# showlab/VideoSwap

Measured on NVIDIA H100. Metric: denoise-steps/sec, 16f 512^2 SD1.5 UNet3D (CFG UNet fwd + CFG combine + DDIM step), higher is better.
Workload: dtype f16

## Files before the change

### videoswap_b200/csrc/common.cuh

```cuda
#pragma once
#include <cuda.h>
#include <cuda_fp16.h>
#include <cuda_runtime.h>
#include <stdint.h>
#include <stdio.h>

namespace vs {

void set_error(const char* fmt, ...);
const char* last_error();

#define VS_CHECK_CUDA(expr)                                                                         \
  do {                                                                                              \
    cudaError_t _e = (expr);                                                                        \
    if (_e != cudaSuccess) {                                                                        \
      vs::set_error("%s:%d CUDA error %s: %s", __FILE__, __LINE__, #expr, cudaGetErrorString(_e)); \
      return 1;                                                                                     \
    }                                                                                               \
  } while (0)

#define VS_REQUIRE(cond, ...)                \
  do {                                       \
    if (!(cond)) {                           \
      vs::set_error(__VA_ARGS__);            \
      return 2;                              \
    }                                        \
  } while (0)

int make_tmap_f16(CUtensorMap* out, const void* base, int rank, const uint64_t* dims, const uint64_t* strides_bytes,
                  const uint32_t* box, int swizzle );

int num_sms();
int get_option(const char* name);

#ifdef __CUDACC__
template <typename... KArgs, typename... Args>
int launch_pdl(void (*kernel)(KArgs...), dim3 grid, dim3 block, size_t smem, cudaStream_t st, int cluster_x, Args&&... args) {
  cudaLaunchConfig_t cfg = {};
  cfg.gridDim = grid;
  cfg.blockDim = block;
  cfg.dynamicSmemBytes = smem;
  cfg.stream = st;
  cudaLaunchAttribute attr[2];
  int n = 0;
  if (get_option("pdl") != 0) {
    attr[n].id = cudaLaunchAttributeProgrammaticStreamSerialization;
    attr[n].val.programmaticStreamSerializationAllowed = 1;
    ++n;
  }
  if (cluster_x > 1) {
    attr[n].id = cudaLaunchAttributeClusterDimension;
    attr[n].val.clusterDim.x = cluster_x;
    attr[n].val.clusterDim.y = 1;
    attr[n].val.clusterDim.z = 1;
    ++n;
  }
  cfg.attrs = attr;
  cfg.numAttrs = n;
  VS_CHECK_CUDA(cudaLaunchKernelEx(&cfg, kernel, static_cast<KArgs>(args)...));
  return 0;
}
#endif

enum ProfCat { PC_GEMM = 0, PC_CONV = 1, PC_ATTN = 2, PC_TATTN = 3, PC_GROUPNORM = 4, PC_LAYERNORM = 5, PC_OTHER = 6, PC_COUNT = 7 };
struct ProfScope {
  ProfScope(cudaStream_t st, int cat, double work, int nlaunch = 1, long long m = 0, int n = 0, int k = 0);
  ~ProfScope();
  cudaStream_t st_; int idx_;
};
void prof_enable(bool on);
void prof_reset();
int prof_collect(int cat, double* ms, double* work, long long* count);
int prof_dump(const char* path);
long long launch_count();
void count_launch(int n);

#ifdef __CUDACC__
__device__ __forceinline__ uint32_t smem_u32(const void* p) { return (uint32_t)__cvta_generic_to_shared(p); }

__device__ __forceinline__ void mbar_init(uint32_t bar, uint32_t count) {
  asm volatile("mbarrier.init.shared::cta.b64 [%0], %1;" ::"r"(bar), "r"(count) : "memory");
}
__device__ __forceinline__ void fence_barrier_init() {
  asm volatile("fence.mbarrier_init.release.cluster;" ::: "memory");
}
__device__ __forceinline__ void fence_proxy_async() { asm volatile("fence.proxy.async.shared::cta;" ::: "memory"); }
__device__ __forceinline__ void mbar_expect_tx(uint32_t bar, uint32_t bytes) {
  asm volatile("mbarrier.arrive.expect_tx.shared::cta.b64 _, [%0], %1;" ::"r"(bar), "r"(bytes) : "memory");
}
__device__ __forceinline__ void mbar_arrive(uint32_t bar) {
  asm volatile("mbarrier.arrive.shared::cta.b64 _, [%0];" ::"r"(bar) : "memory");
}
__device__ __forceinline__ bool mbar_try_wait(uint32_t bar, uint32_t parity) {
  uint32_t ok;
  asm volatile(
      "{\n\t.reg .pred p;\n\t"
      "mbarrier.try_wait.parity.shared::cta.b64 p, [%1], %2;\n\t"
      "selp.u32 %0, 1, 0, p;\n\t}"
      : "=r"(ok)
      : "r"(bar), "r"(parity)
      : "memory");
  return ok != 0;
}
__device__ __forceinline__ void mbar_wait(uint32_t bar, uint32_t parity) {
  if (mbar_try_wait(bar, parity)) return;
  uint32_t spins = 0;
  while (!mbar_try_wait(bar, parity)) {
    if (++spins > (1u << 25)) __trap();
  }
}

__device__ __forceinline__ void prefetch_tmap(const CUtensorMap* m) {
  asm volatile("prefetch.tensormap [%0];" ::"l"(reinterpret_cast<uint64_t>(m)) : "memory");
}
__device__ __forceinline__ void tma_load_2d(uint32_t dst, const CUtensorMap* m, uint32_t bar, int c0, int c1) {
  asm volatile(
      "cp.async.bulk.tensor.2d.shared::cluster.global.mbarrier::complete_tx::bytes [%0], [%1, {%3, %4}], [%2];"
      ::"r"(dst), "l"(reinterpret_cast<uint64_t>(m)), "r"(bar), "r"(c0), "r"(c1)
      : "memory");
}
__device__ __forceinline__ void tma_load_4d(uint32_t dst, const CUtensorMap* m, uint32_t bar, int c0, int c1, int c2,
                                            int c3) {
  asm volatile(
      "cp.async.bulk.tensor.4d.shared::cluster.global.mbarrier::complete_tx::bytes [%0], [%1, {%3, %4, %5, %6}], [%2];"
      ::"r"(dst), "l"(reinterpret_cast<uint64_t>(m)), "r"(bar), "r"(c0), "r"(c1), "r"(c2), "r"(c3)
      : "memory");
}

__device__ __forceinline__ bool elect_one() {
  uint32_t pred;
  asm volatile(
      "{\n\t.reg .pred P;\n\t"
      "elect.sync _|P, 0xffffffff;\n\t"
      "selp.u32 %0, 1, 0, P;\n\t}"
      : "=r"(pred));
  return pred != 0;
}

__device__ __forceinline__ uint32_t cluster_ctarank() {
  uint32_t r;
  asm volatile("mov.u32 %0, %%cluster_ctarank;" : "=r"(r));
  return r;
}
__device__ __forceinline__ void cluster_sync_all() {
  asm volatile("barrier.cluster.arrive.release.aligned;" ::: "memory");
  asm volatile("barrier.cluster.wait.acquire.aligned;" ::: "memory");
}
__device__ __forceinline__ uint32_t mapa_shared(uint32_t addr, uint32_t rank) {
  uint32_t r;
  asm volatile("mapa.shared::cluster.u32 %0, %1, %2;" : "=r"(r) : "r"(addr), "r"(rank));
  return r;
}
__device__ __forceinline__ void named_bar_sync(int id, int nthreads) {
  asm volatile("bar.sync %0, %1;" ::"r"(id), "r"(nthreads) : "memory");
}
__device__ __forceinline__ void named_bar_arrive(int id, int nthreads) {
  asm volatile("bar.arrive %0, %1;" ::"r"(id), "r"(nthreads) : "memory");
}

__device__ __forceinline__ void pdl_trigger() { asm volatile("griddepcontrol.launch_dependents;" ::: "memory"); }
__device__ __forceinline__ void pdl_wait() { asm volatile("griddepcontrol.wait;" ::: "memory"); }

template <int N>
__device__ __forceinline__ void setmaxnreg_dec() { asm volatile("setmaxnreg.dec.sync.aligned.u32 %0;" ::"n"(N)); }
template <int N>
__device__ __forceinline__ void setmaxnreg_inc() { asm volatile("setmaxnreg.inc.sync.aligned.u32 %0;" ::"n"(N)); }

__device__ __forceinline__ void wgmma_fence() { asm volatile("wgmma.fence.sync.aligned;" ::: "memory"); }
__device__ __forceinline__ void wgmma_commit() { asm volatile("wgmma.commit_group.sync.aligned;" ::: "memory"); }
template <int N>
__device__ __forceinline__ void wgmma_wait() { asm volatile("wgmma.wait_group.sync.aligned %0;" ::"n"(N) : "memory"); }

__device__ __forceinline__ uint64_t gmma_desc_sw128(uint32_t smem_addr) {
  uint64_t d = 0;
  d |= (uint64_t)((smem_addr & 0x3FFFF) >> 4);
  d |= (uint64_t)1 << 16;
  d |= (uint64_t)(1024 >> 4) << 32;
  d |= (uint64_t)1 << 62;
  return d;
}
__device__ __forceinline__ uint64_t gmma_desc_sw128_mn(uint32_t smem_addr, uint32_t lbo_bytes) {
  uint64_t d = 0;
  d |= (uint64_t)((smem_addr & 0x3FFFF) >> 4);
  d |= (uint64_t)((lbo_bytes >> 4) & 0x3FFF) << 16;
  d |= (uint64_t)(1024 >> 4) << 32;
  d |= (uint64_t)1 << 62;
  return d;
}

#define VS_R8(i) "+f"(d[i]), "+f"(d[i + 1]), "+f"(d[i + 2]), "+f"(d[i + 3]), "+f"(d[i + 4]), "+f"(d[i + 5]), "+f"(d[i + 6]), "+f"(d[i + 7])
template <int N>
__device__ __forceinline__ void wgmma_ss(float* d, uint64_t da, uint64_t db, uint32_t scale_d);
#define VS_REGS_0_31 "%0,%1,%2,%3,%4,%5,%6,%7,%8,%9,%10,%11,%12,%13,%14,%15,%16,%17,%18,%19,%20,%21,%22,%23,%24,%25,%26,%27,%28,%29,%30,%31"
#define VS_REGS_32_63 "%32,%33,%34,%35,%36,%37,%38,%39,%40,%41,%42,%43,%44,%45,%46,%47,%48,%49,%50,%51,%52,%53,%54,%55,%56,%57,%58,%59,%60,%61,%62,%63"
#define VS_REGS_64_79 "%64,%65,%66,%67,%68,%69,%70,%71,%72,%73,%74,%75,%76,%77,%78,%79"
#define VS_REGS_80_127 "%80,%81,%82,%83,%84,%85,%86,%87,%88,%89,%90,%91,%92,%93,%94,%95,%96,%97,%98,%99,%100,%101,%102,%103,%104,%105,%106,%107,%108,%109,%110,%111,%112,%113,%114,%115,%116,%117,%118,%119,%120,%121,%122,%123,%124,%125,%126,%127"
#define VS_WGMMA_SS(N, REGS, IA, IB, IS, ...)                                                                     \
  template <>                                                                                                     \
  __device__ __forceinline__ void wgmma_ss<N>(float* d, uint64_t da, uint64_t db, uint32_t scale_d) {           \
    asm volatile("{\n\t.reg .pred p;\n\tsetp.ne.b32 p, %" #IS ", 0;\n\t"                                         \
                 "wgmma.mma_async.sync.aligned.m64n" #N "k16.f32.f16.f16 {" REGS "}, %" #IA ", %" #IB ", p, 1, 1, 0, 0;\n\t}" \
                 : __VA_ARGS__                                                                                    \
                 : "l"(da), "l"(db), "r"(scale_d));                                                               \
  }
VS_WGMMA_SS(64, VS_REGS_0_31, 32, 33, 34, VS_R8(0), VS_R8(8), VS_R8(16), VS_R8(24))
VS_WGMMA_SS(128, VS_REGS_0_31 "," VS_REGS_32_63, 64, 65, 66, VS_R8(0), VS_R8(8), VS_R8(16), VS_R8(24), VS_R8(32), VS_R8(40),
            VS_R8(48), VS_R8(56))
VS_WGMMA_SS(160, VS_REGS_0_31 "," VS_REGS_32_63 "," VS_REGS_64_79, 80, 81, 82, VS_R8(0), VS_R8(8), VS_R8(16), VS_R8(24),
            VS_R8(32), VS_R8(40), VS_R8(48), VS_R8(56), VS_R8(64), VS_R8(72))
VS_WGMMA_SS(256, VS_REGS_0_31 "," VS_REGS_32_63 "," VS_REGS_64_79 "," VS_REGS_80_127, 128, 129, 130, VS_R8(0), VS_R8(8),
            VS_R8(16), VS_R8(24), VS_R8(32), VS_R8(40), VS_R8(48), VS_R8(56), VS_R8(64), VS_R8(72), VS_R8(80), VS_R8(88),
            VS_R8(96), VS_R8(104), VS_R8(112), VS_R8(120))
#undef VS_WGMMA_SS
#undef VS_REGS_0_31
#undef VS_REGS_32_63
#undef VS_REGS_64_79
#undef VS_REGS_80_127
template <int TB = 0>
__device__ __forceinline__ void wgmma_m64n16(float* d, uint64_t da, uint64_t db, uint32_t scale_d) {
  asm volatile(
      "{\n\t.reg .pred p;\n\tsetp.ne.b32 p, %10, 0;\n\t"
      "wgmma.mma_async.sync.aligned.m64n16k16.f32.f16.f16 {%0,%1,%2,%3,%4,%5,%6,%7}, %8, %9, p, 1, 1, 0, %11;\n\t}"
      : VS_R8(0)
      : "l"(da), "l"(db), "r"(scale_d), "n"(TB));
}
template <int TB = 0>
__device__ __forceinline__ void wgmma_m64n64_rs(float* d, const uint32_t* a, uint64_t db, uint32_t scale_d) {
  asm volatile(
      "{\n\t.reg .pred p;\n\tsetp.ne.b32 p, %37, 0;\n\t"
      "wgmma.mma_async.sync.aligned.m64n64k16.f32.f16.f16 "
      "{%0,%1,%2,%3,%4,%5,%6,%7,%8,%9,%10,%11,%12,%13,%14,%15,%16,%17,%18,%19,%20,%21,%22,%23,%24,%25,%26,%27,%28,%29,%30,%31}, "
      "{%32,%33,%34,%35}, %36, p, 1, 1, %38;\n\t}"
      : VS_R8(0), VS_R8(8), VS_R8(16), VS_R8(24)
      : "r"(a[0]), "r"(a[1]), "r"(a[2]), "r"(a[3]), "l"(db), "r"(scale_d), "n"(TB));
}
template <int TB = 0>
__device__ __forceinline__ void wgmma_m64n16_rs(float* d, const uint32_t* a, uint64_t db, uint32_t scale_d) {
  asm volatile(
      "{\n\t.reg .pred p;\n\tsetp.ne.b32 p, %13, 0;\n\t"
      "wgmma.mma_async.sync.aligned.m64n16k16.f32.f16.f16 {%0,%1,%2,%3,%4,%5,%6,%7}, {%8,%9,%10,%11}, %12, p, 1, 1, %14;\n\t}"
      : VS_R8(0)
      : "r"(a[0]), "r"(a[1]), "r"(a[2]), "r"(a[3]), "l"(db), "r"(scale_d), "n"(TB));
}
#undef VS_R8

__device__ __forceinline__ float silu_f(float x) { return __fdividef(x, 1.f + __expf(-x)); }
__device__ __forceinline__ float gelu_erf_f(float x) { return 0.5f * x * (1.f + erff(x * 0.70710678118654752f)); }
__device__ __forceinline__ float gelu_erf_fast(float x) {
  const float z = fabsf(x) * 0.70710678118654752f;
  float t;
  asm("rcp.approx.ftz.f32 %0, %1;" : "=f"(t) : "f"(fmaf(0.3275911f, z, 1.f)));
  float poly = fmaf(1.061405429f, t, -1.453152027f);
  poly = fmaf(poly, t, 1.421413741f);
  poly = fmaf(poly, t, -0.284496736f);
  poly = fmaf(poly, t, 0.254829592f);
  poly *= t;
  float e;
  asm("ex2.approx.ftz.f32 %0, %1;" : "=f"(e) : "f"(-1.4426950408889634f * z * z));
  const float erf_abs = fmaf(-poly, e, 1.f);
  const float erf_s = copysignf(erf_abs, x);
  return 0.5f * x * (1.f + erf_s);
}
__device__ __forceinline__ float gelu_sig(float x) {
  const float xc = fminf(fmaxf(x, -5.f), 5.f);
  const float u = xc * xc;
  float q = fmaf(u, 2.47135360e-05f, 7.37690930e-04f);
  q = fmaf(q, u, -1.05988323e-01f);
  q = fmaf(q, u, -2.30164247e+00f);
  float e;
  asm("ex2.approx.ftz.f32 %0, %1;" : "=f"(e) : "f"(xc * q));
  return __fdividef(x, 1.f + e);
}
#endif

}
```

### videoswap_b200/csrc/gemm.cu

```cuda
#include "common.cuh"
#include "kernels.h"

namespace vs {

namespace {

constexpr int BM = 128;
constexpr int WG_M = 64;
constexpr int BK = 64;
constexpr int A_STAGE_BYTES = BM * BK * 2;
constexpr uint64_t A_HALF_DESC = (WG_M * BK * 2) >> 4;
constexpr int GEMM_THREADS = 384;
constexpr int SMEM_LIMIT = 227 * 1024;
constexpr int EPI_COLS = 32;
constexpr int EPI_WARP_BYTES = 16 * 64;
constexpr int EPI_BYTES = 8 * EPI_WARP_BYTES;
constexpr int PRODUCER_REGS = 40, CONSUMER_REGS = 232;
enum { EPI_F_GEGLU = 1, EPI_F_RES = 2, EPI_F_RV = 4, EPI_F_LN = 8, EPI_F_LNOUT = 16 };

struct GemmParams {
  CUtensorMap tmA, tmA2, tmB;
  int M, N;
  int num_kb;
  int kb_per_tap;
  int kb_src1;
  int taps;
  int a_rank;
  int nimg, H, W, TH, TW, TN, tiles_x, tiles_y;
  int tap_x0, tap_y0, tap_w;
  int osy, osx, ooy, oox, OH, OW;
  int tw_log, thw_log;
  int m_tiles, n_tiles;
  const float* bias;
  const float* rowvec;
  int ldrv;
  int pix_per_batch;
  int rv_mod;
  const float2* ln_stats;
  const float* ln_u;
  const float2* ln_parts;
  int ln_nparts;
  float ln_inv_c;
  float2* ln_sums_out;
  const __half* residual;
  int ldr;
  __half* out;
  int ldc;
  int staged;
  int stages;
};

template <int BN>
struct Cfg {
  static constexpr bool COOP = BN > 160;
  static constexpr int HALVES = COOP ? 1 : 2;
  static constexpr int B_STAGE_BYTES = BN * BK * 2;
  static constexpr int STAGE_BYTES = A_STAGE_BYTES + B_STAGE_BYTES;
  static constexpr int STAGES_RAW = (SMEM_LIMIT - 2048 - EPI_BYTES) / STAGE_BYTES;
  static constexpr int STAGES = STAGES_RAW > 12 ? 12 : STAGES_RAW;
  static constexpr int SMEM_BYTES = STAGES * STAGE_BYTES + EPI_BYTES + 1024  + 256 ;
  static_assert(B_STAGE_BYTES % 1024 == 0, "B stage must keep 1024-byte alignment for SWIZZLE_128B");
  static_assert(STAGES >= 3, "pipeline too shallow");
  static_assert(BN % 32 == 0 && BN <= 256, "wgmma N");
};

__device__ __forceinline__ uint32_t sw64_off(int row, int chunk) {
  return (uint32_t)(row * 64 + ((chunk ^ ((row >> 1) & 3)) << 4));
}

template <int BN, int EPI>
__global__ void __launch_bounds__(GEMM_THREADS, 1) gemm_tc_kernel(const __grid_constant__ GemmParams p) {
  using C = Cfg<BN>;
  constexpr bool GEGLU = (EPI & EPI_F_GEGLU) != 0, HAS_RES = (EPI & EPI_F_RES) != 0, HAS_RV = (EPI & EPI_F_RV) != 0;
  constexpr bool LN = (EPI & EPI_F_LN) != 0;
  constexpr bool LNOUT = (EPI & EPI_F_LNOUT) != 0;
  extern __shared__ uint8_t smem_raw[];
  const uint32_t smem_base = (smem_u32(smem_raw) + 1023u) & ~1023u;
  const uint32_t epi_base = smem_base + C::STAGES * C::STAGE_BYTES;
  const uint32_t bar_base = epi_base + EPI_BYTES;
  auto full_bar = [&](int s) { return bar_base + 8u * s; };
  auto empty_bar = [&](int s) { return bar_base + 8u * (C::STAGES + s); };

  const int warp = threadIdx.x >> 5;
  const int lane = threadIdx.x & 31;
  const int wg = threadIdx.x >> 7;
  const int nst = (p.stages > 0 && p.stages < C::STAGES) ? p.stages : C::STAGES;
  const int total_tiles = p.m_tiles * p.n_tiles;

  if (threadIdx.x == 0) {
    prefetch_tmap(&p.tmA);
    prefetch_tmap(&p.tmB);
    if (p.kb_src1 < p.kb_per_tap) prefetch_tmap(&p.tmA2);
    for (int s = 0; s < C::STAGES; ++s) {
      mbar_init(full_bar(s), 1);
      mbar_init(empty_bar(s), C::COOP ? 8 : 4);
    }
    fence_barrier_init();
  }
  __syncthreads();
  pdl_trigger();
  pdl_wait();

  if (wg == 0) {
    setmaxnreg_dec<PRODUCER_REGS>();
    if (warp != 0) return;
    const int num_kb = p.num_kb, kb_per_tap = p.kb_per_tap, kb_src1 = p.kb_src1;
    const bool conv = p.a_rank == 4;
    const int tap_x0 = p.tap_x0, tap_x1 = p.tap_x0 + p.tap_w;
    uint32_t pr_s = 0, pr_ph = 0;
    for (int t = blockIdx.x; t < total_tiles; t += gridDim.x) {
      const int m_tile = t / p.n_tiles, n_tile = t % p.n_tiles;
      int x0 = 0, y0 = 0, i0 = 0;
      if (conv) {
        x0 = (m_tile % p.tiles_x) * p.TW;
        y0 = ((m_tile / p.tiles_x) % p.tiles_y) * p.TH;
        i0 = (m_tile / (p.tiles_x * p.tiles_y)) * p.TN;
      }
      const int n0 = n_tile * BN;
      const int m0 = m_tile * BM;
      int kcoord = 0;
      int dy = p.tap_y0, dx = tap_x0;
      int r = 0;
      for (int kb = 0; kb < num_kb; ++kb) {
        mbar_wait(empty_bar(pr_s), pr_ph ^ 1);
        if (elect_one()) {
          const uint32_t fb = full_bar(pr_s);
          const uint32_t a_dst = smem_base + pr_s * C::STAGE_BYTES;
          const bool first = r < kb_src1;
          const CUtensorMap* tm = first ? &p.tmA : &p.tmA2;
          const int c = (first ? r : r - kb_src1) * BK;
          mbar_expect_tx(fb, C::STAGE_BYTES);
          if (conv) tma_load_4d(a_dst, tm, fb, c, x0 + dx, y0 + dy, i0);
          else tma_load_2d(a_dst, tm, fb, c, m0);
          tma_load_2d(a_dst + A_STAGE_BYTES, &p.tmB, fb, kcoord, n0);
        }
        __syncwarp();
        kcoord += BK;
        if (++r == kb_per_tap) {
          r = 0;
          if (++dx == tap_x1) { dx = tap_x0; ++dy; }
        }
        if (++pr_s == (uint32_t)nst) { pr_s = 0; pr_ph ^= 1; }
      }
    }
    return;
  }

  setmaxnreg_inc<CONSUMER_REGS>();
  const int g = wg - 1;
  const int wq = warp & 3;
  const int q = lane & 3;
  const int rbase = 16 * wq + (lane >> 2);
  const uint32_t stage_buf = epi_base + (uint32_t)(warp - 4) * EPI_WARP_BYTES;
  const bool has_bias = p.bias != nullptr;
  const bool staged = p.staged != 0;
  const int num_kb = p.num_kb;
  auto tile_pixel = [&](int m_tile, int row) -> int {
    if (p.a_rank == 4) {
      const int x0 = (m_tile % p.tiles_x) * p.TW;
      const int y0 = ((m_tile / p.tiles_x) % p.tiles_y) * p.TH;
      const int i0 = (m_tile / (p.tiles_x * p.tiles_y)) * p.TN;
      const int ti = row >> p.thw_log, rem = row & ((1 << p.thw_log) - 1);
      const int y = y0 + (rem >> p.tw_log), x = x0 + (rem & (p.TW - 1)), img = i0 + ti;
      return ((img < p.nimg) && (y < p.H) && (x < p.W)) ? (img * p.OH + y * p.osy + p.ooy) * p.OW + x * p.osx + p.oox : -1;
    }
    const int px = m_tile * BM + row;
    return px < p.M ? px : -1;
  };

  const int bar_mine = 1 + g, bar_other = 2 - g;
  float acc[C::HALVES][BN / 2];
  uint32_t s = 0, ph = 0;
  for (int t = blockIdx.x, j = 0; t < total_tiles; t += gridDim.x, ++j) {
    const int m_tile = t / p.n_tiles, n_tile = t % p.n_tiles;
    if (!C::COOP && (j & 1) != g) {
      const uint32_t sn = s + (uint32_t)num_kb;
      ph ^= (sn / (uint32_t)nst) & 1u;
      s = sn % (uint32_t)nst;
      continue;
    }
    if (!C::COOP && j > 0) named_bar_sync(bar_mine, 256);
    uint32_t prev = 0;
    for (int kb = 0; kb < num_kb; ++kb) {
      mbar_wait(full_bar(s), ph);
      wgmma_fence();
      const uint32_t a_addr = smem_base + s * C::STAGE_BYTES;
      const uint64_t da = gmma_desc_sw128(a_addr) + (C::COOP ? (uint64_t)g * A_HALF_DESC : 0);
      const uint64_t db = gmma_desc_sw128(a_addr + A_STAGE_BYTES);
#pragma unroll
      for (int k = 0; k < BK / 16; ++k) {
#pragma unroll
        for (int hh = 0; hh < C::HALVES; ++hh)
          wgmma_ss<BN>(acc[hh], da + hh * A_HALF_DESC + 2 * k, db + 2 * k, (kb | k) != 0 ? 1u : 0u);
      }
      wgmma_commit();
      if (kb > 0) {
        wgmma_wait<1>();
        if (lane == 0) mbar_arrive(empty_bar(prev));
      }
      prev = s;
      if (++s == (uint32_t)nst) { s = 0; ph ^= 1; }
    }
    if (!C::COOP && t + (int)gridDim.x < total_tiles) named_bar_arrive(bar_other, 256);
    wgmma_wait<0>();
    if (lane == 0) mbar_arrive(empty_bar(prev));

    const int n0 = n_tile * BN;
#pragma unroll
    for (int hh = 0; hh < C::HALVES; ++hh) {
      const int r0 = WG_M * (C::COOP ? g : hh) + rbase;
      int pix[2];
      pix[0] = tile_pixel(m_tile, r0);
      pix[1] = tile_pixel(m_tile, r0 + 8);
      const float* rv[2] = {nullptr, nullptr};
      if (HAS_RV || !staged) {
#pragma unroll
        for (int h = 0; h < 2; ++h) {
          if (p.rowvec != nullptr && pix[h] >= 0) {
            int ri = pix[h] / p.pix_per_batch;
            if (p.rv_mod > 0) ri %= p.rv_mod;
            rv[h] = p.rowvec + (long long)ri * p.ldrv + n0;
          }
        }
      }
      if (staged) {
        constexpr int OC = GEGLU ? BN / 2 : BN;
        const int oc0 = n_tile * OC;
        const int nsub = (p.N - n0 < BN ? (GEGLU ? (p.N - n0) / 2 : p.N - n0) : OC) / EPI_COLS;
        float la[2] = {1.f, 1.f}, lb[2] = {0.f, 0.f};
        if (LN) {
#pragma unroll
          for (int h = 0; h < 2; ++h) {
            if (pix[h] < 0) continue;
            if (p.ln_nparts > 0) {
              float S = 0.f, Q = 0.f;
              for (int k = 0; k < p.ln_nparts; ++k) {
                const float2 v = __ldg(p.ln_parts + (long long)k * p.M + pix[h]);
                S += v.x; Q += v.y;
              }
              const float mean = S * p.ln_inv_c;
              la[h] = rsqrtf(fmaxf(fmaf(-mean, mean, Q * p.ln_inv_c), 0.f) + 1e-5f);
              lb[h] = -mean * la[h];
            } else {
              const float2 st2 = __ldg(p.ln_stats + pix[h]);
              la[h] = st2.x; lb[h] = st2.y;
            }
          }
        }
        float rs[2] = {0.f, 0.f}, rq[2] = {0.f, 0.f};
        __half* orow[2];
        const __half* rrow[2];
#pragma unroll
        for (int h = 0; h < 2; ++h) {
          const long long px = pix[h] >= 0 ? pix[h] : 0;
          orow[h] = p.out + px * p.ldc + oc0 + q * 8;
          rrow[h] = HAS_RES ? p.residual + px * p.ldr + oc0 + q * 8 : nullptr;
        }
#pragma unroll
        for (int sb = 0; sb < OC / EPI_COLS; ++sb) {
          if (sb >= nsub) break;
          uint4 rr[2];
          if (HAS_RES) {
#pragma unroll
            for (int h = 0; h < 2; ++h) rr[h] = __ldg(reinterpret_cast<const uint4*>(rrow[h] + sb * EPI_COLS));
          }
#pragma unroll
          for (int jj = 0; jj < 4; ++jj) {
            const int j = 4 * sb + jj;
            const int c = 8 * j + 2 * q;
            float2 b = has_bias ? __ldg(reinterpret_cast<const float2*>(p.bias + n0 + c)) : make_float2(0.f, 0.f);
            float2 u = LN ? __ldg(reinterpret_cast<const float2*>(p.ln_u + n0 + c)) : make_float2(0.f, 0.f);
            float2 bg = make_float2(0.f, 0.f), ug = make_float2(0.f, 0.f);
            if (GEGLU) {
              bg = __ldg(reinterpret_cast<const float2*>(p.bias + n0 + BN / 2 + c));
              if (LN) ug = __ldg(reinterpret_cast<const float2*>(p.ln_u + n0 + BN / 2 + c));
            }
#pragma unroll
            for (int h = 0; h < 2; ++h) {
              float f0 = acc[hh][4 * j + 2 * h], f1 = acc[hh][4 * j + 2 * h + 1];
              if (GEGLU) {
                float g0 = acc[hh][4 * (j + BN / 16) + 2 * h], g1 = acc[hh][4 * (j + BN / 16) + 2 * h + 1];
                float bv0 = b.x, bv1 = b.y, bg0 = bg.x, bg1 = bg.y;
                if (LN) {
                  bv0 = fmaf(lb[h], u.x, bv0); bv1 = fmaf(lb[h], u.y, bv1);
                  bg0 = fmaf(lb[h], ug.x, bg0); bg1 = fmaf(lb[h], ug.y, bg1);
                  f0 *= la[h]; f1 *= la[h]; g0 *= la[h]; g1 *= la[h];
                }
                f0 = (f0 + bv0) * gelu_sig(g0 + bg0);
                f1 = (f1 + bv1) * gelu_sig(g1 + bg1);
              } else {
                if (LN) {
                  f0 = fmaf(la[h], f0, fmaf(lb[h], u.x, b.x));
                  f1 = fmaf(la[h], f1, fmaf(lb[h], u.y, b.y));
                } else if (has_bias) {
                  f0 += b.x; f1 += b.y;
                }
                if (HAS_RV && rv[h] != nullptr) {
                  const float2 r2 = __ldg(reinterpret_cast<const float2*>(rv[h] + c));
                  f0 += r2.x; f1 += r2.y;
                }
              }
              const __half2 hv = __floats2half2_rn(f0, f1);
              asm volatile("st.shared.b32 [%0], %1;" ::"r"(stage_buf + sw64_off((lane >> 2) + 8 * h, jj) + 4 * q),
                           "r"(*reinterpret_cast<const uint32_t*>(&hv)) : "memory");
            }
          }
          __syncwarp();
#pragma unroll
          for (int h = 0; h < 2; ++h) {
            uint4 o;
            asm volatile("ld.shared.v4.b32 {%0,%1,%2,%3}, [%4];" : "=r"(o.x), "=r"(o.y), "=r"(o.z), "=r"(o.w)
                         : "r"(stage_buf + sw64_off((lane >> 2) + 8 * h, q)));
            if (HAS_RES) {
              __half2* oh = reinterpret_cast<__half2*>(&o);
              const __half2* rh = reinterpret_cast<const __half2*>(&rr[h]);
#pragma unroll
              for (int t = 0; t < 4; ++t) oh[t] = __hadd2(oh[t], rh[t]);
            }
            if (pix[h] >= 0) *reinterpret_cast<uint4*>(orow[h] + sb * EPI_COLS) = o;
            if (LNOUT) {
              const __half2* oh = reinterpret_cast<const __half2*>(&o);
              const float2 a = __half22float2(oh[0]), b2 = __half22float2(oh[1]), c2 = __half22float2(oh[2]), d2 = __half22float2(oh[3]);
              rs[h] += ((a.x + a.y) + (b2.x + b2.y)) + ((c2.x + c2.y) + (d2.x + d2.y));
              float q0 = fmaf(a.x, a.x, a.y * a.y), q1 = fmaf(b2.x, b2.x, b2.y * b2.y);
              float q2 = fmaf(c2.x, c2.x, c2.y * c2.y), q3 = fmaf(d2.x, d2.x, d2.y * d2.y);
              rq[h] += (q0 + q1) + (q2 + q3);
            }
          }
          __syncwarp();
        }
        if (LNOUT) {
#pragma unroll
          for (int h = 0; h < 2; ++h) {
            rs[h] += __shfl_xor_sync(0xffffffffu, rs[h], 1); rq[h] += __shfl_xor_sync(0xffffffffu, rq[h], 1);
            rs[h] += __shfl_xor_sync(0xffffffffu, rs[h], 2); rq[h] += __shfl_xor_sync(0xffffffffu, rq[h], 2);
            if (q == 0 && pix[h] >= 0) p.ln_sums_out[(long long)n_tile * p.M + pix[h]] = make_float2(rs[h], rq[h]);
          }
        }
      } else {
#pragma unroll
        for (int j = 0; j < BN / 8; ++j) {
#pragma unroll
          for (int e = 0; e < 4; ++e) {
            const int h = e >> 1, c = 8 * j + 2 * q + (e & 1), n = n0 + c;
            if (n < p.N && pix[h] >= 0) {
              float f = acc[hh][4 * j + e];
              if (has_bias) f += p.bias[n];
              if (rv[h]) f += rv[h][c];
              if (p.residual) f += __half2float(p.residual[(long long)pix[h] * p.ldr + n]);
              p.out[(long long)pix[h] * p.ldc + n] = __float2half_rn(f);
            }
          }
        }
      }
    }
  }
}

struct ConvTile { int tw, th, tn; };

ConvTile pick_conv_tile(int nimg, int H, int W) {
  ConvTile best{1, 1, BM};
  long long best_cost = -1;
  for (int tw = 1; tw <= BM; tw *= 2) {
    for (int th = 1; tw * th <= BM; th *= 2) {
      const int tn = BM / (tw * th);
      if (tw > 256 || th > 256 || tn > 256) continue;
      const long long cost = (long long)((W + tw - 1) / tw) * tw * ((H + th - 1) / th) * th * ((nimg + tn - 1) / tn) * tn;
      if (best_cost < 0 || cost < best_cost || (cost == best_cost && tw > best.tw)) {
        best_cost = cost;
        best = ConvTile{tw, th, tn};
      }
    }
  }
  return best;
}

template <int BN, int EPI>
int launch(cudaStream_t st, const GemmParams& p) {
  using C = Cfg<BN>;
  static bool configured = false;
  if (!configured) {
    VS_CHECK_CUDA(cudaFuncSetAttribute(gemm_tc_kernel<BN, EPI>, cudaFuncAttributeMaxDynamicSharedMemorySize, C::SMEM_BYTES));
    configured = true;
  }
  const int total = p.m_tiles * p.n_tiles;
  int ctas = num_sms();
  const int cap = get_option("gemm_ctas");
  if (cap > 0 && cap < ctas) ctas = cap;
  return launch_pdl(gemm_tc_kernel<BN, EPI>, dim3(total < ctas ? total : ctas), dim3(GEMM_THREADS), C::SMEM_BYTES, st, 1, p);
}

template <int BN>
int launch_linear(cudaStream_t st, const GemmParams& p) {
  const int epi = (p.residual ? EPI_F_RES : 0) | (p.rowvec ? EPI_F_RV : 0) | ((p.ln_stats || p.ln_parts) ? EPI_F_LN : 0) |
                  (p.ln_sums_out ? EPI_F_LNOUT : 0);
  switch (epi) {
    case EPI_F_LNOUT: return launch<BN, EPI_F_LNOUT>(st, p);
    case EPI_F_LNOUT | EPI_F_RES: return launch<BN, EPI_F_LNOUT | EPI_F_RES>(st, p);
    case EPI_F_LN: return launch<BN, EPI_F_LN>(st, p);
    case EPI_F_LN | EPI_F_RV: return launch<BN, EPI_F_LN | EPI_F_RV>(st, p);
    case 0: return launch<BN, 0>(st, p);
    case EPI_F_RES: return launch<BN, EPI_F_RES>(st, p);
    case EPI_F_RV: return launch<BN, EPI_F_RV>(st, p);
    case EPI_F_RES | EPI_F_RV: return launch<BN, EPI_F_RES | EPI_F_RV>(st, p);
    default: set_error("gemm_tc: unsupported epilogue combination 0x%x", epi); return 2;
  }
}

int pick_bn(int m_tiles, int N, int num_kb) {
  if (N <= 64) return 64;
  int best = 128;
  long long best_cost = -1;
  const int cand[3] = {128, 160, 256};
  for (int i = 0; i < 3; ++i) {
    const int bn = cand[i];
    if (bn != 128 && N % bn != 0) continue;
    const long long tiles = (long long)m_tiles * ((N + bn - 1) / bn);
    const long long waves = (tiles + num_sms() - 1) / num_sms();
    const long long cost = waves * (16 + bn / 8);
    if (best_cost < 0 || cost < best_cost || (cost == best_cost && num_kb >= 40)) {
      best_cost = cost;
      best = bn;
    }
  }
  return best;
}

int ilog2(int v) { int l = 0; while ((1 << l) < v) ++l; return l; }

}

int gemm_n_tiles(const GemmArgs& a) {
  if (a.taps != 1) return 0;
  int bn = a.force_bn;
  if (a.mode == EPI_GEGLU) bn = 2 * kGegluGranule;
  else if (bn == 0) bn = pick_bn((a.M + BM - 1) / BM, a.N, (a.K1 + BK - 1) / BK + a.K2 / BK);
  return (a.N + bn - 1) / bn;
}

int gemm_tc(cudaStream_t st, const GemmArgs& a) {
  VS_REQUIRE(a.A && a.Bw && a.out, "gemm_tc: null pointer");
  VS_REQUIRE(a.taps == 1 || a.taps == 9 || a.taps == 4, "gemm_tc: taps must be 1, 9 (3x3) or 4 (2x2 sub-pixel)");
  VS_REQUIRE(a.K1 % 8 == 0 && a.K2 % 8 == 0, "gemm_tc: K must be a multiple of 8 (TMA 16-byte strides)");
  VS_REQUIRE((long long)a.M * (a.ldc > a.ldr ? a.ldc : a.ldr) < (1LL << 40) && a.M < (1 << 30), "gemm_tc: M too large");
  const bool two = a.A2 != nullptr && a.K2 > 0;
  if (two || a.taps != 1) VS_REQUIRE(a.K1 % BK == 0 && a.K2 % BK == 0, "gemm_tc: concat/conv sources need C %% 64 == 0 (got %d,%d)", a.K1, a.K2);
  GemmParams p;
  memset(&p, 0, sizeof(p));
  const int Ktap = a.K1 + (two ? a.K2 : 0);
  const int Ktot = Ktap * a.taps;
  p.taps = a.taps;
  p.kb_src1 = (a.K1 + BK - 1) / BK;
  p.kb_per_tap = p.kb_src1 + (two ? a.K2 / BK : 0);
  p.num_kb = p.kb_per_tap * a.taps;
  p.M = a.M;
  p.N = a.N;
  p.bias = a.bias;
  p.rowvec = a.rowvec;
  p.ldrv = a.ldrv > 0 ? a.ldrv : a.N;
  p.pix_per_batch = a.pix_per_batch > 0 ? a.pix_per_batch : 1;
  p.rv_mod = a.rv_mod;
  p.ln_stats = reinterpret_cast<const float2*>(a.ln_stats);
  p.ln_u = a.ln_u;
  p.ln_parts = reinterpret_cast<const float2*>(a.ln_parts);
  p.ln_nparts = a.ln_parts ? a.ln_nparts : 0;
  p.ln_inv_c = 1.f / (float)(a.K1 + a.K2);
  p.ln_sums_out = reinterpret_cast<float2*>(a.ln_sums_out);
  if (a.ln_parts) VS_REQUIRE(a.ln_stats == nullptr && a.ln_nparts >= 1 && a.ln_nparts <= 16 && a.taps == 1, "gemm_tc: bad LayerNorm partial-sum input");
  if (a.ln_stats || a.ln_parts) VS_REQUIRE(a.ln_u != nullptr && a.bias != nullptr && a.residual == nullptr, "gemm_tc: folded LayerNorm needs u and c vectors and no residual");
  if (a.ln_sums_out) VS_REQUIRE(a.taps == 1 && a.mode == EPI_LINEAR && a.rowvec == nullptr && !a.ln_stats && !a.ln_parts,
                                "gemm_tc: row statistics output is implemented for plain linear layers (+ bias / residual)");
  p.residual = a.residual;
  p.ldr = a.ldr;
  p.out = a.out;
  p.ldc = a.ldc;
  p.stages = get_option("gemm_stages");

  if (a.taps != 1) {
    VS_REQUIRE(a.nimg > 0 && a.H > 0 && a.W > 0 && a.M == a.nimg * a.H * a.W, "gemm_tc: bad conv geometry");
    p.a_rank = 4;
    if (a.taps == 9) { p.tap_x0 = p.tap_y0 = -1; p.tap_w = 3; p.osy = p.osx = 1; p.ooy = p.oox = 0; p.OH = a.H; p.OW = a.W; }
    else {
      VS_REQUIRE((a.sub_py | 1) == 1 && (a.sub_px | 1) == 1, "gemm_tc: sub-pixel parity must be 0 or 1");
      p.tap_y0 = a.sub_py - 1; p.tap_x0 = a.sub_px - 1; p.tap_w = 2;
      p.osy = p.osx = 2; p.ooy = a.sub_py; p.oox = a.sub_px; p.OH = 2 * a.H; p.OW = 2 * a.W;
    }
    const ConvTile t = pick_conv_tile(a.nimg, a.H, a.W);
    p.nimg = a.nimg; p.H = a.H; p.W = a.W; p.TW = t.tw; p.TH = t.th; p.TN = t.tn;
    p.tw_log = ilog2(t.tw);
    p.thw_log = ilog2(t.tw * t.th);
    p.tiles_x = (a.W + t.tw - 1) / t.tw;
    p.tiles_y = (a.H + t.th - 1) / t.th;
    p.m_tiles = p.tiles_x * p.tiles_y * ((a.nimg + t.tn - 1) / t.tn);
    const uint32_t box[4] = {BK, (uint32_t)t.tw, (uint32_t)t.th, (uint32_t)t.tn};
    {
      const uint64_t dims[4] = {(uint64_t)a.K1, (uint64_t)a.W, (uint64_t)a.H, (uint64_t)a.nimg};
      const uint64_t str[3] = {(uint64_t)a.lda1 * 2, (uint64_t)a.lda1 * 2 * a.W, (uint64_t)a.lda1 * 2 * a.W * a.H};
      if (make_tmap_f16(&p.tmA, a.A, 4, dims, str, box, 1)) return 3;
    }
    if (two) {
      const uint64_t dims[4] = {(uint64_t)a.K2, (uint64_t)a.W, (uint64_t)a.H, (uint64_t)a.nimg};
      const uint64_t str[3] = {(uint64_t)a.lda2 * 2, (uint64_t)a.lda2 * 2 * a.W, (uint64_t)a.lda2 * 2 * a.W * a.H};
      if (make_tmap_f16(&p.tmA2, a.A2, 4, dims, str, box, 1)) return 3;
    }
  } else {
    p.a_rank = 2;
    p.m_tiles = (a.M + BM - 1) / BM;
    const uint32_t box[2] = {BK, BM};
    {
      const uint64_t dims[2] = {(uint64_t)a.K1, (uint64_t)a.M};
      const uint64_t str[1] = {(uint64_t)a.lda1 * 2};
      if (make_tmap_f16(&p.tmA, a.A, 2, dims, str, box, 1)) return 3;
    }
    if (two) {
      const uint64_t dims[2] = {(uint64_t)a.K2, (uint64_t)a.M};
      const uint64_t str[1] = {(uint64_t)a.lda2 * 2};
      if (make_tmap_f16(&p.tmA2, a.A2, 2, dims, str, box, 1)) return 3;
    }
  }

  int bn = a.force_bn;
  if (a.mode == EPI_GEGLU) {
    bn = 2 * kGegluGranule;
    VS_REQUIRE(a.N % bn == 0, "gemm_tc: GEGLU needs N %% %d == 0 (N=%d)", bn, a.N);
    VS_REQUIRE(a.bias != nullptr && a.residual == nullptr && a.rowvec == nullptr, "gemm_tc: GEGLU takes a bias only");
  } else if (bn == 0) {
    bn = pick_bn(p.m_tiles, a.N, p.num_kb);
  }
  VS_REQUIRE(bn == 64 || bn == 128 || bn == 160 || bn == 256, "gemm_tc: unsupported BLOCK_N %d", bn);
  p.n_tiles = (a.N + bn - 1) / bn;
  {
    const uint64_t dims[2] = {(uint64_t)Ktot, (uint64_t)a.N};
    const uint64_t str[1] = {(uint64_t)Ktot * 2};
    const uint32_t box[2] = {BK, (uint32_t)bn};
    if (make_tmap_f16(&p.tmB, a.Bw, 2, dims, str, box, 1)) return 3;
  }
  const int out_cols = (a.mode == EPI_GEGLU) ? a.N / 2 : a.N;
  p.staged = (out_cols % EPI_COLS == 0) && (a.ldc % 8 == 0) && ((reinterpret_cast<uintptr_t>(a.out) & 15) == 0) &&
             (!a.residual || ((a.ldr % 8 == 0) && ((reinterpret_cast<uintptr_t>(a.residual) & 15) == 0))) &&
             (!a.bias || (reinterpret_cast<uintptr_t>(a.bias) & 15) == 0) &&
             (!a.rowvec || ((reinterpret_cast<uintptr_t>(a.rowvec) & 15) == 0 && p.ldrv % 4 == 0));
  if (!p.staged) VS_REQUIRE(a.mode == EPI_LINEAR, "gemm_tc: GEGLU output needs 32-column aligned, 16-byte strided rows");
  if (a.ln_stats || a.ln_parts) VS_REQUIRE(p.staged && (reinterpret_cast<uintptr_t>(a.ln_u) & 15) == 0, "gemm_tc: folded LayerNorm needs the staged epilogue");
  if (a.ln_sums_out) VS_REQUIRE(p.staged, "gemm_tc: row statistics output needs the staged epilogue (N %% 32 == 0, aligned rows)");
  ProfScope prof(st, a.taps != 1 ? PC_CONV : PC_GEMM, 2.0 * a.M * (double)a.N * Ktot, 1, a.M, a.N, Ktot);
  if (a.mode == EPI_GEGLU) {
    if (p.ln_stats || p.ln_parts) return launch<256, EPI_F_GEGLU | EPI_F_LN>(st, p);
    return launch<256, EPI_F_GEGLU>(st, p);
  }
  switch (bn) {
    case 64: return launch_linear<64>(st, p);
    case 128: return launch_linear<128>(st, p);
    case 256: return launch_linear<256>(st, p);
    default: return launch_linear<160>(st, p);
  }
}

}
```

Before: 10.92.

## Use TMA loads and stores for residual-add GEMM epilogue

For linear GEMMs with a residual on ping-pong tiles, the residual is now prefetched into shared memory by TMA while the mainloop runs. The output is written back with TMA bulk tensor stores from per-warpgroup staging buffers, replacing per-thread global loads and stores. The staging buffer grows to a full 64xBN tile per warpgroup, which can cut pipeline stages. The change also stops choosing BN=256 for short K loops and drops the gemm_stages runtime option.

```diff
diff --git a/videoswap_b200/csrc/common.cuh b/videoswap_b200/csrc/common.cuh
--- a/videoswap_b200/csrc/common.cuh
+++ b/videoswap_b200/csrc/common.cuh
@@ -119,6 +119,13 @@
       ::"r"(dst), "l"(reinterpret_cast<uint64_t>(m)), "r"(bar), "r"(c0), "r"(c1)
       : "memory");
 }
+__device__ __forceinline__ void tma_store_2d(const CUtensorMap* m, uint32_t src, int c0, int c1) {
+  asm volatile("cp.async.bulk.tensor.2d.global.shared::cta.bulk_group [%0, {%2, %3}], [%1];"
+               ::"l"(reinterpret_cast<uint64_t>(m)), "r"(src), "r"(c0), "r"(c1)
+               : "memory");
+}
+__device__ __forceinline__ void bulk_commit() { asm volatile("cp.async.bulk.commit_group;" ::: "memory"); }
+__device__ __forceinline__ void bulk_wait_read_all() { asm volatile("cp.async.bulk.wait_group.read 0;" ::: "memory"); }
 __device__ __forceinline__ void tma_load_4d(uint32_t dst, const CUtensorMap* m, uint32_t bar, int c0, int c1, int c2,
                                             int c3) {
   asm volatile(
diff --git a/videoswap_b200/csrc/gemm.cu b/videoswap_b200/csrc/gemm.cu
--- a/videoswap_b200/csrc/gemm.cu
+++ b/videoswap_b200/csrc/gemm.cu
@@ -14,12 +14,15 @@
 constexpr int SMEM_LIMIT = 227 * 1024;
 constexpr int EPI_COLS = 32;
 constexpr int EPI_WARP_BYTES = 16 * 64;
-constexpr int EPI_BYTES = 8 * EPI_WARP_BYTES;
+constexpr int EPI_BOX_BYTES = WG_M * 64;
+constexpr int TMA_EPI_MAX_BN = 160;
+constexpr int MAX_STAGES = 12;
 constexpr int PRODUCER_REGS = 40, CONSUMER_REGS = 232;
-enum { EPI_F_GEGLU = 1, EPI_F_RES = 2, EPI_F_RV = 4, EPI_F_LN = 8, EPI_F_LNOUT = 16 };
+enum { EPI_F_GEGLU = 1, EPI_F_RES = 2, EPI_F_RV = 4, EPI_F_LN = 8, EPI_F_LNOUT = 16, EPI_F_TMA = 32 };
 
 struct GemmParams {
   CUtensorMap tmA, tmA2, tmB;
+  CUtensorMap tmOut, tmRes;
   int M, N;
   int num_kb;
   int kb_per_tap;
@@ -47,19 +50,26 @@
   __half* out;
   int ldc;
   int staged;
+  int tma_out;
   int stages;
 };
 
-template <int BN>
+template <int BN, int EPI = 0>
 struct Cfg {
   static constexpr bool COOP = BN > 160;
   static constexpr int HALVES = COOP ? 1 : 2;
+  static constexpr int OC = (EPI & EPI_F_GEGLU) ? BN / 2 : BN;
+  static constexpr bool TMA = (EPI & EPI_F_TMA) != 0;
   static constexpr int B_STAGE_BYTES = BN * BK * 2;
   static constexpr int STAGE_BYTES = A_STAGE_BYTES + B_STAGE_BYTES;
-  static constexpr int STAGES_RAW = (SMEM_LIMIT - 2048 - EPI_BYTES) / STAGE_BYTES;
-  static constexpr int STAGES = STAGES_RAW > 12 ? 12 : STAGES_RAW;
-  static constexpr int SMEM_BYTES = STAGES * STAGE_BYTES + EPI_BYTES + 1024  + 256 ;
+  static constexpr int CBUF_BYTES = TMA ? WG_M * OC * 2 : 4 * EPI_WARP_BYTES;
+  static constexpr int STAGES_RAW = (SMEM_LIMIT - 2048 - 2 * CBUF_BYTES) / STAGE_BYTES;
+  static constexpr int STAGES = STAGES_RAW > MAX_STAGES ? MAX_STAGES : STAGES_RAW;
+  static constexpr int SMEM_BYTES = STAGES * STAGE_BYTES + 2 * CBUF_BYTES + 1024  + 256 ;
   static_assert(B_STAGE_BYTES % 1024 == 0, "B stage must keep 1024-byte alignment for SWIZZLE_128B");
+  static_assert(CBUF_BYTES % 1024 == 0, "staging must keep 1024-byte alignment for the swizzled TMA boxes");
+  static_assert(!TMA || (!COOP && !(EPI & EPI_F_GEGLU) && (EPI & EPI_F_RES)),
+                "the TMA-store epilogue is for ping-pong linear tiles with a residual");
   static_assert(STAGES >= 3, "pipeline too shallow");
   static_assert(BN % 32 == 0 && BN <= 256, "wgmma N");
 };
@@ -70,16 +80,19 @@
 
 template <int BN, int EPI>
 __global__ void __launch_bounds__(GEMM_THREADS, 1) gemm_tc_kernel(const __grid_constant__ GemmParams p) {
-  using C = Cfg<BN>;
+  using C = Cfg<BN, EPI>;
   constexpr bool GEGLU = (EPI & EPI_F_GEGLU) != 0, HAS_RES = (EPI & EPI_F_RES) != 0, HAS_RV = (EPI & EPI_F_RV) != 0;
   constexpr bool LN = (EPI & EPI_F_LN) != 0;
   constexpr bool LNOUT = (EPI & EPI_F_LNOUT) != 0;
+  constexpr int OC = C::OC;
+  constexpr bool tma_out = C::TMA;
   extern __shared__ uint8_t smem_raw[];
   const uint32_t smem_base = (smem_u32(smem_raw) + 1023u) & ~1023u;
   const uint32_t epi_base = smem_base + C::STAGES * C::STAGE_BYTES;
-  const uint32_t bar_base = epi_base + EPI_BYTES;
+  const uint32_t bar_base = epi_base + 2 * C::CBUF_BYTES;
   auto full_bar = [&](int s) { return bar_base + 8u * s; };
   auto empty_bar = [&](int s) { return bar_base + 8u * (C::STAGES + s); };
+  auto res_bar = [&](int g) { return bar_base + 8u * (2 * C::STAGES + g); };
 
   const int warp = threadIdx.x >> 5;
   const int lane = threadIdx.x & 31;
@@ -91,9 +104,17 @@
     prefetch_tmap(&p.tmA);
     prefetch_tmap(&p.tmB);
     if (p.kb_src1 < p.kb_per_tap) prefetch_tmap(&p.tmA2);
+    if (tma_out) {
+      prefetch_tmap(&p.tmOut);
+      prefetch_tmap(&p.tmRes);
+    }
     for (int s = 0; s < C::STAGES; ++s) {
       mbar_init(full_bar(s), 1);
       mbar_init(empty_bar(s), C::COOP ? 8 : 4);
+    }
+    if (tma_out) {
+      mbar_init(res_bar(0), 1);
+      mbar_init(res_bar(1), 1);
     }
     fence_barrier_init();
   }
@@ -151,7 +172,10 @@
   const int wq = warp & 3;
   const int q = lane & 3;
   const int rbase = 16 * wq + (lane >> 2);
-  const uint32_t stage_buf = epi_base + (uint32_t)(warp - 4) * EPI_WARP_BYTES;
+  const uint32_t cbuf = epi_base + (uint32_t)g * C::CBUF_BYTES;
+  const uint32_t wbuf = cbuf + (uint32_t)wq * EPI_WARP_BYTES;
+  constexpr uint32_t sb_stride = tma_out ? EPI_BOX_BYTES : 0;
+  const bool leader = (threadIdx.x & 127) == 0;
   const bool has_bias = p.bias != nullptr;
   const bool staged = p.staged != 0;
   const int num_kb = p.num_kb;
@@ -167,6 +191,20 @@
     const int px = m_tile * BM + row;
     return px < p.M ? px : -1;
   };
+  auto half_row0 = [&](int hh) { return WG_M * (C::COOP ? g : hh); };
+  auto tile_nsub = [&](int n_tile) {
+    const int n0 = n_tile * BN;
+    return (p.N - n0 < BN ? (GEGLU ? (p.N - n0) / 2 : p.N - n0) : OC) / EPI_COLS;
+  };
+  auto half_live = [&](int m_tile, int hh) { return m_tile * BM + half_row0(hh) < p.M; };
+  uint32_t res_ph = 0;
+  auto load_residual = [&](int m_tile, int n_tile, int hh) {
+    bulk_wait_read_all();
+    const int nsub = tile_nsub(n_tile);
+    mbar_expect_tx(res_bar(g), nsub * EPI_BOX_BYTES);
+    for (int sb = 0; sb < nsub; ++sb)
+      tma_load_2d(cbuf + sb * EPI_BOX_BYTES, &p.tmRes, res_bar(g), n_tile * OC + sb * EPI_COLS, m_tile * BM + half_row0(hh));
+  };
 
   const int bar_mine = 1 + g, bar_other = 2 - g;
   float acc[C::HALVES][BN / 2];
@@ -179,6 +217,7 @@
       s = sn % (uint32_t)nst;
       continue;
     }
+    if (tma_out && leader && half_live(m_tile, 0)) load_residual(m_tile, n_tile, 0);
     if (!C::COOP && j > 0) named_bar_sync(bar_mine, 256);
     uint32_t prev = 0;
     for (int kb = 0; kb < num_kb; ++kb) {
@@ -208,7 +247,12 @@
     const int n0 = n_tile * BN;
 #pragma unroll
     for (int hh = 0; hh < C::HALVES; ++hh) {
-      const int r0 = WG_M * (C::COOP ? g : hh) + rbase;
+      if (tma_out) {
+        if (!half_live(m_tile, hh)) continue;
+        mbar_wait(res_bar(g), res_ph);
+        res_ph ^= 1;
+      }
+      const int r0 = half_row0(hh) + rbase;
       int pix[2];
       pix[0] = tile_pixel(m_tile, r0);
       pix[1] = tile_pixel(m_tile, r0 + 8);
@@ -224,9 +268,8 @@
         }
       }
       if (staged) {
-        constexpr int OC = GEGLU ? BN / 2 : BN;
         const int oc0 = n_tile * OC;
-        const int nsub = (p.N - n0 < BN ? (GEGLU ? (p.N - n0) / 2 : p.N - n0) : OC) / EPI_COLS;
+        const int nsub = tile_nsub(n_tile);
         float la[2] = {1.f, 1.f}, lb[2] = {0.f, 0.f};
         if (LN) {
 #pragma unroll
@@ -250,17 +293,20 @@
         float rs[2] = {0.f, 0.f}, rq[2] = {0.f, 0.f};
         __half* orow[2];
         const __half* rrow[2];
-#pragma unroll
-        for (int h = 0; h < 2; ++h) {
-          const long long px = pix[h] >= 0 ? pix[h] : 0;
-          orow[h] = p.out + px * p.ldc + oc0 + q * 8;
-          rrow[h] = HAS_RES ? p.residual + px * p.ldr + oc0 + q * 8 : nullptr;
+        if (!tma_out) {
+#pragma unroll
+          for (int h = 0; h < 2; ++h) {
+            const long long px = pix[h] >= 0 ? pix[h] : 0;
+            orow[h] = p.out + px * p.ldc + oc0 + q * 8;
+            rrow[h] = HAS_RES ? p.residual + px * p.ldr + oc0 + q * 8 : nullptr;
+          }
         }
 #pragma unroll
         for (int sb = 0; sb < OC / EPI_COLS; ++sb) {
           if (sb >= nsub) break;
+          const uint32_t sbuf = wbuf + sb * sb_stride;
           uint4 rr[2];
-          if (HAS_RES) {
+          if (HAS_RES && !tma_out) {
 #pragma unroll
             for (int h = 0; h < 2; ++h) rr[h] = __ldg(reinterpret_cast<const uint4*>(rrow[h] + sb * EPI_COLS));
           }
@@ -300,24 +346,31 @@
                   f0 += r2.x; f1 += r2.y;
                 }
               }
-              const __half2 hv = __floats2half2_rn(f0, f1);
-              asm volatile("st.shared.b32 [%0], %1;" ::"r"(stage_buf + sw64_off((lane >> 2) + 8 * h, jj) + 4 * q),
-                           "r"(*reinterpret_cast<const uint32_t*>(&hv)) : "memory");
+              __half2 hv = __floats2half2_rn(f0, f1);
+              const uint32_t addr = sbuf + sw64_off((lane >> 2) + 8 * h, jj) + 4 * q;
+              if (HAS_RES && tma_out) {
+                uint32_t r;
+                asm volatile("ld.shared.b32 %0, [%1];" : "=r"(r) : "r"(addr));
+                hv = __hadd2(hv, *reinterpret_cast<const __half2*>(&r));
+              }
+              asm volatile("st.shared.b32 [%0], %1;" ::"r"(addr), "r"(*reinterpret_cast<const uint32_t*>(&hv)) : "memory");
             }
           }
           __syncwarp();
 #pragma unroll
-          for (int h = 0; h < 2; ++h) {
+          for (int h = 0; h < 2 && (!tma_out || LNOUT); ++h) {
             uint4 o;
             asm volatile("ld.shared.v4.b32 {%0,%1,%2,%3}, [%4];" : "=r"(o.x), "=r"(o.y), "=r"(o.z), "=r"(o.w)
-                         : "r"(stage_buf + sw64_off((lane >> 2) + 8 * h, q)));
-            if (HAS_RES) {
-              __half2* oh = reinterpret_cast<__half2*>(&o);
-              const __half2* rh = reinterpret_cast<const __half2*>(&rr[h]);
-#pragma unroll
-              for (int t = 0; t < 4; ++t) oh[t] = __hadd2(oh[t], rh[t]);
+                         : "r"(sbuf + sw64_off((lane >> 2) + 8 * h, q)));
+            if (!tma_out) {
+              if (HAS_RES) {
+                __half2* oh = reinterpret_cast<__half2*>(&o);
+                const __half2* rh = reinterpret_cast<const __half2*>(&rr[h]);
+#pragma unroll
+                for (int t = 0; t < 4; ++t) oh[t] = __hadd2(oh[t], rh[t]);
+              }
+              if (pix[h] >= 0) *reinterpret_cast<uint4*>(orow[h] + sb * EPI_COLS) = o;
             }
-            if (pix[h] >= 0) *reinterpret_cast<uint4*>(orow[h] + sb * EPI_COLS) = o;
             if (LNOUT) {
               const __half2* oh = reinterpret_cast<const __half2*>(&o);
               const float2 a = __half22float2(oh[0]), b2 = __half22float2(oh[1]), c2 = __half22float2(oh[2]), d2 = __half22float2(oh[3]);
@@ -328,6 +381,16 @@
             }
           }
           __syncwarp();
+        }
+        if (tma_out) {
+          fence_proxy_async();
+          named_bar_sync(3 + g, 128);
+          if (leader) {
+            const int row0 = m_tile * BM + half_row0(hh);
+            for (int sb = 0; sb < nsub; ++sb) tma_store_2d(&p.tmOut, cbuf + sb * EPI_BOX_BYTES, oc0 + sb * EPI_COLS, row0);
+            bulk_commit();
+            if (HAS_RES && hh + 1 < C::HALVES && half_live(m_tile, hh + 1)) load_residual(m_tile, n_tile, hh + 1);
+          }
         }
         if (LNOUT) {
 #pragma unroll
@@ -354,6 +417,7 @@
         }
       }
     }
+    if (tma_out && leader && t + 2 * (int)gridDim.x >= total_tiles) bulk_wait_read_all();
   }
 }
 
@@ -378,7 +442,7 @@
 
 template <int BN, int EPI>
 int launch(cudaStream_t st, const GemmParams& p) {
-  using C = Cfg<BN>;
+  using C = Cfg<BN, EPI>;
   static bool configured = false;
   if (!configured) {
     VS_CHECK_CUDA(cudaFuncSetAttribute(gemm_tc_kernel<BN, EPI>, cudaFuncAttributeMaxDynamicSharedMemorySize, C::SMEM_BYTES));
@@ -393,17 +457,20 @@
 
 template <int BN>
 int launch_linear(cudaStream_t st, const GemmParams& p) {
+  constexpr int TMA = BN <= TMA_EPI_MAX_BN ? EPI_F_TMA : 0;
   const int epi = (p.residual ? EPI_F_RES : 0) | (p.rowvec ? EPI_F_RV : 0) | ((p.ln_stats || p.ln_parts) ? EPI_F_LN : 0) |
                   (p.ln_sums_out ? EPI_F_LNOUT : 0);
+  const bool tma = p.tma_out;
   switch (epi) {
     case EPI_F_LNOUT: return launch<BN, EPI_F_LNOUT>(st, p);
-    case EPI_F_LNOUT | EPI_F_RES: return launch<BN, EPI_F_LNOUT | EPI_F_RES>(st, p);
+    case EPI_F_LNOUT | EPI_F_RES:
+      return tma ? launch<BN, EPI_F_LNOUT | EPI_F_RES | TMA>(st, p) : launch<BN, EPI_F_LNOUT | EPI_F_RES>(st, p);
     case EPI_F_LN: return launch<BN, EPI_F_LN>(st, p);
     case EPI_F_LN | EPI_F_RV: return launch<BN, EPI_F_LN | EPI_F_RV>(st, p);
     case 0: return launch<BN, 0>(st, p);
-    case EPI_F_RES: return launch<BN, EPI_F_RES>(st, p);
+    case EPI_F_RES: return tma ? launch<BN, EPI_F_RES | TMA>(st, p) : launch<BN, EPI_F_RES>(st, p);
     case EPI_F_RV: return launch<BN, EPI_F_RV>(st, p);
-    case EPI_F_RES | EPI_F_RV: return launch<BN, EPI_F_RES | EPI_F_RV>(st, p);
+    case EPI_F_RES | EPI_F_RV: return tma ? launch<BN, EPI_F_RES | EPI_F_RV | TMA>(st, p) : launch<BN, EPI_F_RES | EPI_F_RV>(st, p);
     default: set_error("gemm_tc: unsupported epilogue combination 0x%x", epi); return 2;
   }
 }
@@ -416,6 +483,7 @@
   for (int i = 0; i < 3; ++i) {
     const int bn = cand[i];
     if (bn != 128 && N % bn != 0) continue;
+    if (bn == 256 && num_kb < 40) continue;
     const long long tiles = (long long)m_tiles * ((N + bn - 1) / bn);
     const long long waves = (tiles + num_sms() - 1) / num_sms();
     const long long cost = waves * (16 + bn / 8);
@@ -475,7 +543,6 @@
   p.ldr = a.ldr;
   p.out = a.out;
   p.ldc = a.ldc;
-  p.stages = get_option("gemm_stages");
 
   if (a.taps != 1) {
     VS_REQUIRE(a.nimg > 0 && a.H > 0 && a.W > 0 && a.M == a.nimg * a.H * a.W, "gemm_tc: bad conv geometry");
@@ -544,6 +611,15 @@
   if (!p.staged) VS_REQUIRE(a.mode == EPI_LINEAR, "gemm_tc: GEGLU output needs 32-column aligned, 16-byte strided rows");
   if (a.ln_stats || a.ln_parts) VS_REQUIRE(p.staged && (reinterpret_cast<uintptr_t>(a.ln_u) & 15) == 0, "gemm_tc: folded LayerNorm needs the staged epilogue");
   if (a.ln_sums_out) VS_REQUIRE(p.staged, "gemm_tc: row statistics output needs the staged epilogue (N %% 32 == 0, aligned rows)");
+  p.tma_out = p.staged && p.a_rank == 2 && a.mode == EPI_LINEAR && bn <= TMA_EPI_MAX_BN && a.residual != nullptr &&
+              (long long)p.m_tiles * p.n_tiles > num_sms();
+  if (p.tma_out) {
+    const uint32_t box[2] = {EPI_COLS, WG_M};
+    const uint64_t dims[2] = {(uint64_t)out_cols, (uint64_t)a.M};
+    const uint64_t str_out[1] = {(uint64_t)a.ldc * 2}, str_res[1] = {(uint64_t)a.ldr * 2};
+    if (make_tmap_f16(&p.tmOut, a.out, 2, dims, str_out, box, 2)) return 3;
+    if (make_tmap_f16(&p.tmRes, a.residual, 2, dims, str_res, box, 2)) return 3;
+  }
   ProfScope prof(st, a.taps != 1 ? PC_CONV : PC_GEMM, 2.0 * a.M * (double)a.N * Ktot, 1, a.M, a.N, Ktot);
   if (a.mode == EPI_GEGLU) {
     if (p.ln_stats || p.ln_parts) return launch<256, EPI_F_GEGLU | EPI_F_LN>(st, p);
```

Result: no change. 10.95 (median of 6 runs) (+0.3%).
